# mantasu/face-crop-plus

Measured on AMD Instinct MI355X. Metric: faces/sec end-to-end (detect+align+crop), higher is better.
Workload: dtype f16x3; 1 GPU; RetinaFace detect + 5-pt align/crop, batch=32/GPU synthetic 1024x1024 RGB, strategy=largest, det_threshold=0.6, output 256x256, detector on 2 HIP streams x 16 images; global_batch=32, image_size=1024, parallelism=dp1

## Files before the change

### face-crop-plus_amd/csrc/fcp_bneck_chain.hip

```cpp
#include "fcp_conv_common.h"

#include <type_traits>

using namespace fcp_conv;

namespace {

typedef _Float16 f16x8 __attribute__((ext_vector_type(8)));

constexpr int FCP_CHAIN_STORE_AUX = 2;

struct ChainK {
  const float* t1;  unsigned t1_bytes;  int t1_ld;
  const float* w2;  unsigned w2_bytes;  const float* ws2;  const float* b2;
  const float* w3;  unsigned w3_bytes;  const float* ws3;  const float* b3;
  const float* res; int res_ld;
  float* out;       int out_ld;    unsigned out_bytes;
  const float* w1n; unsigned w1n_bytes; const float* ws1n; const float* b1n;
  float* t1n;       int t1n_ld;
  int n, h, w, M;
  int nt_store;
  int out_even;
  const float* t1b; unsigned t1b_bytes; int t1b_ld, hb, wb, sb;
};

constexpr int BMT = 128;
constexpr int C = 64;
constexpr int ROWB = 128;
constexpr int STAGE = (BMT + C) * ROWB;
constexpr int CT_OFF = 0;
constexpr int W1B_OFF = BMT * 128;
constexpr bool w1_double(int cn, bool has_c2) { return !has_c2 || W1B_OFF + 2 * cn * 128 + 2 * C * 128 <= 2 * STAGE; }
constexpr int w3b_off(int cn, bool has_c2) { return W1B_OFF + (w1_double(cn, has_c2) ? 2 : 1) * cn * 128; }
constexpr int r0_bytes(int cw, int cn, bool has_c2) { return has_c2 ? 2 * STAGE : w3b_off(cn, has_c2) + 2 * cw * 128; }
constexpr bool alias_t2(bool has_c2) { return !has_c2; }
constexpr int lds_bytes(int cw, int cn, bool has_c2, bool direct = false) {
  const int r0 = r0_bytes(cw, cn, has_c2), t2 = BMT * cw * 4;
  if (direct) return r0;
  return !alias_t2(has_c2) ? r0 + t2 : (r0 > W1B_OFF + t2 ? r0 : W1B_OFF + t2);
}
constexpr int wgs_per_cu(int cw, int cn, bool has_c2, bool direct = false) {
  if (direct) return cn == 0 && lds_bytes(cw, cn, has_c2, true) <= 80 * 1024 ? 2 : 1;
  return lds_bytes(cw, cn, has_c2) <= 80 * 1024 ? 2 : 1;
}

__device__ __forceinline__ int swz(int row) { return ((row >> 1) & 7) ^ ((row & 1) << 2); }

constexpr bool direct_form(int cn, int cw2) { return cw2 > 0 || cn == 0; }
template <int CN, int CW, int NOUT, bool HAS_C2, bool HAS_RES, int CW2 = 0>
__global__ void __launch_bounds__(2 * BMT, wgs_per_cu(CW, CN, HAS_C2, direct_form(CN, CW2))) bneck_chain_c64(const ChainK p) {
  constexpr bool DIRECT = direct_form(CN, CW2);
  static_assert(!DIRECT || (!HAS_C2 && CW2 % 32 == 0 && CW2 < CW), "direct forms are pair forms");
  constexpr bool HAS_P3 = CN > 0;
  static_assert(!HAS_C2 || CW == C, "phase 1 is written for 64-channel bottlenecks");
  constexpr bool PATCH = HAS_C2;
  constexpr int PH = BMT / 16;
  constexpr int NTHR = 2 * BMT;
  constexpr int NW = NTHR / 64;
  constexpr int LR = NTHR / 8;
  constexpr int TN3 = CN / 32;
  constexpr int TN3A = TN3 > 0 ? TN3 : 1;
  constexpr int CS = CW / 32;
  constexpr int NCH = NOUT / 32;
  constexpr int W3CH = CW * 128;
  constexpr bool ALIAS = alias_t2(HAS_C2) && !DIRECT;
  constexpr int T2_OFF = ALIAS ? W1B_OFF : r0_bytes(CW, CN, HAS_C2);
  constexpr int WGS = wgs_per_cu(CW, CN, HAS_C2, DIRECT);
  constexpr int WPS = WGS * NW / 4;
  static_assert(lds_bytes(CW, CN, HAS_C2, DIRECT) <= 160 * 1024, "LDS budget");
  constexpr bool W1DB = w1_double(CN, HAS_C2);
  constexpr bool SPREAD = W1DB && (HAS_C2 || WPS == 1);
  constexpr bool ROT = false;
  constexpr int PQ = ROT ? TN3 / CS : 0;
  static_assert(!ROT || (TN3 % CS == 0 && PQ >= 1), "rotated loop: TN3 must be a multiple of CS");
  constexpr bool W1PRE = !ROT && W1DB && !DIRECT && (HAS_C2 ? CN <= 64 || WPS == 1 : CN <= 128 && WPS == 1);
  constexpr int W3B_OFF = w3b_off(CN, HAS_C2);
  static_assert(!HAS_C2 || W3B_OFF + 2 * W3CH <= 2 * STAGE, "chunk buffers must fit the phase-1 stage region");
  constexpr int NRES = HAS_RES ? 4 : 0;
  extern __shared__ __attribute__((aligned(16))) float smem[];
  char* lds = reinterpret_cast<char*>(smem);

  const int nb = gridDim.x;
  const int bid = blockIdx.x;
  const int q8 = nb >> 3, r8 = nb & 7, xcd = bid & 7;
  const int tile_m = (xcd < r8 ? xcd * (q8 + 1) : r8 * (q8 + 1) + (xcd - r8) * q8) + (bid >> 3);

  const int tid = threadIdx.x;
  const int lane = tid & 63;
  const int wave = tid >> 6;
  const int wave_u = __builtin_amdgcn_readfirstlane(wave);
  const int lrow = tid >> 3;
  const int csrc = (tid & 7) ^ swz(lrow);
  const int l31 = lane & 31, half = lane >> 5;
  const int rsw = swz(l31);
  int offH[2], offL[2];
#pragma unroll
  for (int s = 0; s < 2; ++s) {
    offH[s] = ((2 * s + half) ^ rsw) << 4;
    offL[s] = ((4 + 2 * s + half) ^ rsw) << 4;
  }
// ... 33 lines not shown
      for (int e = 0; e < 8; ++e) {
        ws8[e] = p.ws2[ccol + e];
        b8[e] = p.b2[ccol + e];
      }
#pragma unroll
      for (int g = 0; g < 4; ++g) {
        const int row = (tid >> 3) + LR * g;
        const f32x4 a = *reinterpret_cast<const f32x4*>(Cs + row * C + ccol);
        const f32x4 b = *reinterpret_cast<const f32x4*>(Cs + row * C + ccol + 4);
        float v[8] = {a[0], a[1], a[2], a[3], b[0], b[1], b[2], b[3]};
#pragma unroll
        for (int e = 0; e < 8; ++e) v[e] = conv_value_relu(v[e], ws8[e], b8[e]);
        u32x4_t hi, lo;
        split8(f32x4{v[0], v[1], v[2], v[3]}, f32x4{v[4], v[5], v[6], v[7]}, hi, lo);
        const int q = (ccol & 31) >> 3, sw = swz(row);
        char* trow = lds + T2_OFF + (ccol >> 5) * (BMT * ROWB) + row * ROWB;
        *reinterpret_cast<u32x4_t*>(trow + ((q ^ sw) << 4)) = hi;
        *reinterpret_cast<u32x4_t*>(trow + (((4 + q) ^ sw) << 4)) = lo;
      }
    }
    __syncthreads();
  };

  if constexpr (HAS_C2) {
    constexpr int HALO = (PH + 2) * 18;
    constexpr int HROWS = (HALO + LR - 1) / LR * LR;
    constexpr int ASL = HROWS * ROWB;
    constexpr int TPB = 2, NSTEP = 18 / TPB;
    static_assert(18 % TPB == 0, "taps per barrier must divide the 18 K slices");
    constexpr int BST_OFF = 2 * ASL, BSL = C * ROWB, BSTG = TPB * BSL;
    static_assert(BST_OFF + 2 * BSTG <= T2_OFF + BMT * C * 4, "halo patch + filter stages must fit region 0 + T2");
    f32x16 acc1[2];
    const int wm = wave / 2, wn = wave % 2;
    __amdgpu_buffer_rsrc_t rs_in = __builtin_amdgcn_make_buffer_rsrc(const_cast<float*>(p.t1), 0, p.t1_bytes, 0x00020000);
    __amdgpu_buffer_rsrc_t rs_w = __builtin_amdgcn_make_buffer_rsrc(const_cast<float*>(p.w2), 0, p.w2_bytes, 0x00020000);
#pragma unroll
    for (int i = 0; i < HROWS / LR; ++i) {
      const int r = lrow + LR * i;
      const int hy = r / 18, hx = r - hy * 18;
      const int y = py0 - 1 + hy, x = px0 - 1 + hx;
      const bool ok = r < HALO && (unsigned)y < (unsigned)p.h && (unsigned)x < (unsigned)p.w;
      const unsigned src = ok ? ((unsigned)((pn * p.h + y) * p.w + x) * (unsigned)p.t1_ld + (unsigned)(csrc * 4)) * 4u : 0xFFFFFFFFu;
#pragma unroll
      for (int cs = 0; cs < 2; ++cs)
        __builtin_amdgcn_raw_ptr_buffer_load_lds(rs_in, (__attribute__((address_space(3))) void*)(lds + cs * ASL + (wave_u * 8 + LR * i) * ROWB), 16,
                                                 (int)(src == 0xFFFFFFFFu ? 0xFFFFFFFFu : src + (unsigned)(cs * 32 * 4)), 0, 0, 0);
    }
    constexpr int B_LD = C / LR;
    unsigned woff[B_LD];
#pragma unroll
    for (int i = 0; i < B_LD; ++i) woff[i] = (unsigned)(((lrow + LR * i) * (9 * C) + csrc * 4) * 4);
    auto dma_b = [&](int step, int stage) {
#pragma unroll
      for (int u = 0; u < TPB; ++u)
#pragma unroll
        for (int i = 0; i < B_LD; ++i)
          __builtin_amdgcn_raw_ptr_buffer_load_lds(rs_w, (__attribute__((address_space(3))) void*)(lds + BST_OFF + stage * BSTG + u * BSL + (wave_u * 8 + LR * i) * ROWB), 16,
                                                   (int)(woff[i] + (unsigned)((step * TPB + u) * BK * 4)), 0, 0, 0);
    };
    dma_b(0, 0);
#pragma unroll
    for (int i = 0; i < 2; ++i)
#pragma unroll
      for (int e = 0; e < 16; ++e) acc1[i][e] = 0.f;
    int hr0[2];
#pragma unroll
    for (int i = 0; i < 2; ++i) hr0[i] = (wm * 4 + i * 2 + (l31 >> 4)) * 18 + (l31 & 15);
    const char* Bw = lds + BST_OFF + (wn * 32 + l31) * ROWB;
    fcp_static_for<0, NSTEP>([&](auto gc) {
      constexpr int g = decltype(gc)::value;
// ... 21 lines not shown
          bl[sq] = *reinterpret_cast<const f16x8*>(Bb + offL[sq]);
        }
        if constexpr (decltype(uc)::value == TPB - 1) {
          asm volatile("s_waitcnt lgkmcnt(0)" ::: "memory");
          __builtin_amdgcn_sched_barrier(0);
          if constexpr (g + 1 < NSTEP) dma_b(g + 1, (g + 1) & 1);
          __builtin_amdgcn_sched_barrier(0);
        }
#pragma unroll
        for (int sq = 0; sq < 2; ++sq)
#pragma unroll
          for (int i = 0; i < 2; ++i) {
            acc1[i] = __builtin_amdgcn_mfma_f32_32x32x16_f16(al[sq][i], bh[sq], acc1[i], 0, 0, 0);
            acc1[i] = __builtin_amdgcn_mfma_f32_32x32x16_f16(ah[sq][i], bl[sq], acc1[i], 0, 0, 0);
            acc1[i] = __builtin_amdgcn_mfma_f32_32x32x16_f16(ah[sq][i], bh[sq], acc1[i], 0, 0, 0);
          }
        __builtin_amdgcn_sched_barrier(0);
      });
    });
    asm volatile("s_waitcnt vmcnt(0)" ::: "memory");
    __builtin_amdgcn_s_barrier();
    __builtin_amdgcn_sched_barrier(0);
    conv2_epilogue(acc1, wm, wn);
  } else if constexpr (!DIRECT) {
    __amdgpu_buffer_rsrc_t rs_in = __builtin_amdgcn_make_buffer_rsrc(const_cast<float*>(p.t1), 0, p.t1_bytes, 0x00020000);
#pragma unroll
    for (int i = 0; i < BMT / LR; ++i) {
      const int m = tile_m * BMT + lrow + LR * i;
      const unsigned ro = m < p.M ? ((unsigned)m * (unsigned)p.t1_ld + (unsigned)(csrc * 4)) * 4u : 0xFFFFFFFFu;
#pragma unroll
      for (int sl = 0; sl < CS; ++sl)
        __builtin_amdgcn_raw_ptr_buffer_load_lds(rs_in, (__attribute__((address_space(3))) void*)(lds + T2_OFF + sl * BMT * ROWB + wave_u * 8 * ROWB + LR * i * ROWB),
                                                 16, (int)(ro == 0xFFFFFFFFu ? 0xFFFFFFFFu : ro + (unsigned)(sl * 128)), 0, 0, 0);
    }
  }

  __amdgpu_buffer_rsrc_t rs_w3 = __builtin_amdgcn_make_buffer_rsrc(const_cast<float*>(p.w3), 0, p.w3_bytes, 0x00020000);
  __amdgpu_buffer_rsrc_t rs_w1 = __builtin_amdgcn_make_buffer_rsrc(const_cast<float*>(p.w1n), 0, p.w1n_bytes, 0x00020000);
  constexpr int PW3 = 4 * CS / NW;
  constexpr int PW1 = CN / (8 * NW);
  static_assert(PW3 >= 1 && (PW1 >= 1 || !HAS_P3), "filter pieces per wave");
  auto dma_w3 = [&](int j, int buf) {
#pragma unroll
    for (int i = 0; i < PW3; ++i) {
      const int g = wave_u * PW3 + i, sl = g >> 2, r = (g & 3) * 8 + (lane >> 3);
      char* dst = lds + W3B_OFF + buf * W3CH + sl * 4096 + (g & 3) * 8 * ROWB;
      const unsigned src = (unsigned)((j * 32 + r) * (CW * 4) + sl * 128 + (((lane & 7) ^ swz(r)) << 4));
      __builtin_amdgcn_raw_ptr_buffer_load_lds(rs_w3, (__attribute__((address_space(3))) void*)dst, 16, (int)src, 0, 0, 0);
    }
  };
  auto dma_w1 = [&](int j, int buf) {
    char* dst = lds + W1B_OFF + buf * (CN * ROWB) + wave_u * (CN / NW) * ROWB;
#pragma unroll
    for (int i = 0; i < PW1; ++i) {
      const int r = wave_u * (CN / NW) + 8 * i + (lane >> 3);
      const unsigned src = (unsigned)(r * (NOUT * 4) + j * 128 + (((lane & 7) ^ swz(r)) << 4));
      __builtin_amdgcn_raw_ptr_buffer_load_lds(rs_w1, (__attribute__((address_space(3))) void*)(dst + 8 * i * ROWB), 16, (int)src, 0, 0, 0);
    }
  };
  constexpr int NDMA = PW3 + PW1;
  auto dma_one = [&](auto kc, int j, int buf) {
    constexpr int k = decltype(kc)::value;
    if constexpr (k < PW3) {
      const int g = wave_u * PW3 + k, sl = g >> 2, r = (g & 3) * 8 + (lane >> 3);
      char* dst = lds + W3B_OFF + buf * W3CH + sl * 4096 + (g & 3) * 8 * ROWB;
      const unsigned src = (unsigned)((j * 32 + r) * (CW * 4) + sl * 128 + (((lane & 7) ^ swz(r)) << 4));
      __builtin_amdgcn_raw_ptr_buffer_load_lds(rs_w3, (__attribute__((address_space(3))) void*)dst, 16, (int)src, 0, 0, 0);
    } else {
      constexpr int i = k - PW3;
      const int j1 = ROT ? j - 1 : j, buf1 = ROT ? (j1 & 1) : buf;
      char* dst = lds + W1B_OFF + buf1 * (CN * ROWB) + wave_u * (CN / NW) * ROWB;
      const int r = wave_u * (CN / NW) + 8 * i + (lane >> 3);
      const unsigned src = (unsigned)(r * (NOUT * 4) + j1 * 128 + (((lane & 7) ^ swz(r)) << 4));
      __builtin_amdgcn_raw_ptr_buffer_load_lds(rs_w1, (__attribute__((address_space(3))) void*)(dst + 8 * i * ROWB), 16, (int)src, 0, 0, 0);
    }
  };

  f32x16 acc3[TN3A];
#pragma unroll
  for (int t = 0; t < TN3; ++t)
#pragma unroll
    for (int e = 0; e < 16; ++e) acc3[t][e] = 0.f;

  const char* a2base = lds + T2_OFF + (wave * 32 + l31) * ROWB;
  const char* a3base = lds + CT_OFF + (wave * 32 + l31) * ROWB;
  const int eq = lane & 3;
  const int erow0 = wave * 32 + (lane >> 2);
  long rm[2];
  unsigned so[2];
// ... 2 lines not shown
    const int prow = erow0 + 16 * it;
    const long m = pix(prow);
    rm[it] = m >= 0 ? m : (long)p.M - 1;
    const bool keep = !PATCH || !p.out_even || ((((prow >> 4) | prow) & 1) == 0);
    so[it] = (m >= 0 && keep) ? (unsigned)(m * p.out_ld * 4 + eq * 16) : 0xFFFFFFFFu;
  }
  __amdgpu_buffer_rsrc_t rs_out = __builtin_amdgcn_make_buffer_rsrc(p.out, 0, p.out_bytes, 0x00020000);

  u32x4_t rhi[2], rlo[2];
  auto load_res = [&](int j) {
    if constexpr (!HAS_RES) return;
#pragma unroll
    for (int it = 0; it < 2; ++it) {
      const char* pb = reinterpret_cast<const char*>(p.res) + rm[it] * p.res_ld * 4 + j * 128 + eq * 16;
      rhi[it] = *reinterpret_cast<const u32x4_t*>(pb);
      rlo[it] = *reinterpret_cast<const u32x4_t*>(pb + 64);
    }
  };
  const int nch = NCH;
  f16x8 pch[2], pcl[2];
  f16x8 wx[ROT ? TN3 : 1], wy[ROT ? TN3 : 1];
  float ws_l = p.ws3[l31], b_l = p.b3[l31];
  constexpr int NCONST = 2;
  f16x8 ah[CS][2], al[CS][2];
  auto read_a2 = [&]() {
#pragma unroll
    for (int sl = 0; sl < CS; ++sl)
#pragma unroll
      for (int s = 0; s < 2; ++s) {
        ah[sl][s] = *reinterpret_cast<const f16x8*>(a2base + sl * BMT * ROWB + offH[s]);
        al[sl][s] = *reinterpret_cast<const f16x8*>(a2base + sl * BMT * ROWB + offL[s]);
      }
  };
  if constexpr (DIRECT) {
    constexpr int CS1 = (CW - CW2) / 32;
    __amdgpu_buffer_rsrc_t rs_a = __builtin_amdgcn_make_buffer_rsrc(const_cast<float*>(p.t1), 0, p.t1_bytes, 0x00020000);
    __amdgpu_buffer_rsrc_t rs_b = __builtin_amdgcn_make_buffer_rsrc(const_cast<float*>(p.t1b), 0, p.t1b_bytes, 0x00020000);
    asm volatile("" ::: "memory");
    dma_w3(0, 0);
    if constexpr (W1DB && !ROT) dma_w1(0, 0);
    asm volatile("" ::: "memory");
    const long m = pix(wave * 32 + l31);
    unsigned oa = 0xFFFFFFFFu, ob = 0xFFFFFFFFu;
    if (m >= 0) {
      const int ni = (int)(m / hw);
      const int rem = (int)(m - (long)ni * hw);
      const int y = rem / p.w, x = rem - y * p.w;
      oa = (unsigned)m * (unsigned)p.t1_ld * 4u;
      ob = ((unsigned)(ni * p.hb + y * p.sb) * (unsigned)p.wb + (unsigned)(x * p.sb)) * (unsigned)p.t1b_ld * 4u;
    }
// ... 5 lines not shown
        const unsigned base = first ? oa : ob;
        const unsigned off = (unsigned)((first ? sl : sl - CS1) * 128);
        const unsigned vh = base == 0xFFFFFFFFu ? base : base + off + (unsigned)((2 * sk + half) << 4);
        const unsigned vl = base == 0xFFFFFFFFu ? base : base + off + (unsigned)((4 + 2 * sk + half) << 4);
        ah[sl][sk] = __builtin_bit_cast(f16x8, __builtin_amdgcn_raw_buffer_load_b128(first ? rs_a : rs_b, (int)vh, 0, 0));
        al[sl][sk] = __builtin_bit_cast(f16x8, __builtin_amdgcn_raw_buffer_load_b128(first ? rs_a : rs_b, (int)vl, 0, 0));
      }
    asm volatile("s_waitcnt vmcnt(0)" ::: "memory");
#pragma unroll
    for (int sl = 0; sl < CS; ++sl)
#pragma unroll
      for (int sk = 0; sk < 2; ++sk) asm volatile("" : "+v"(ah[sl][sk]), "+v"(al[sl][sk]));
    __builtin_amdgcn_sched_barrier(0);
  }
  if constexpr (ALIAS) {
    asm volatile("s_waitcnt vmcnt(0)" ::: "memory");
    __builtin_amdgcn_s_barrier();
    __builtin_amdgcn_sched_barrier(0);
    read_a2();
    asm volatile("s_waitcnt lgkmcnt(0)" ::: "memory");
    __builtin_amdgcn_s_barrier();
    __builtin_amdgcn_sched_barrier(0);
  }
  asm volatile("" ::: "memory");
  if constexpr (!DIRECT) {
    dma_w3(0, 0);
    if constexpr (W1DB && !ROT) dma_w1(0, 0);
  }
  asm volatile("" ::: "memory");
  if (nch > 0) load_res(0);
  __builtin_amdgcn_sched_barrier(0);

  for (int j = 0; j < nch; ++j) {
    const bool more = j + 1 < NCH;
    if (j == 0) asm volatile("s_waitcnt vmcnt(%0)" ::"n"(NRES) : "memory");
    else asm volatile("s_waitcnt vmcnt(%0)" ::"n"(4 + NCONST + NRES) : "memory");
    asm volatile("s_waitcnt lgkmcnt(0)" ::: "memory");
    __builtin_amdgcn_s_barrier();
    __builtin_amdgcn_sched_barrier(0);
    if constexpr (!SPREAD) {
      if (more) dma_w3(j + 1, (j + 1) & 1);
      if constexpr (W1DB) {
        if (more) dma_w1(j + 1, (j + 1) & 1);
      } else {
        dma_w1(j, 0);
      }
    }
    asm volatile("" ::: "memory");
    __builtin_amdgcn_sched_barrier(0);
    const char* b2base = lds + W3B_OFF + (j & 1) * W3CH + l31 * ROWB;
    if constexpr (!ALIAS && !DIRECT) {
      if (j == 0) read_a2();
    }
    constexpr int BG = (CS <= 4 && (HAS_C2 || WPS == 1)) ? CS : 2;
    f16x8 bh[2][BG][2], bl[2][BG][2];
    auto read_b2 = [&](int buf, int g) {
#pragma unroll
      for (int q = 0; q < BG; ++q)
#pragma unroll
        for (int s = 0; s < 2; ++s) {
          bh[buf][q][s] = *reinterpret_cast<const f16x8*>(b2base + (g * BG + q) * 4096 + offH[s]);
          bl[buf][q][s] = *reinterpret_cast<const f16x8*>(b2base + (g * BG + q) * 4096 + offL[s]);
        }
    };
    read_b2(0, 0);
    f16x8 dh[2][TN3A], dl[2][TN3A];
    if constexpr (W1PRE) {
      const char* w1b = lds + W1B_OFF + (j & 1) * (CN * ROWB);
#pragma unroll
      for (int s = 0; s < 2; ++s)
#pragma unroll
        for (int t = 0; t < TN3; ++t) {
          dh[s][t] = *reinterpret_cast<const f16x8*>(w1b + (t * 32 + l31) * ROWB + offH[s]);
          dl[s][t] = *reinterpret_cast<const f16x8*>(w1b + (t * 32 + l31) * ROWB + offL[s]);
// ... 210 lines not shown
      const f32x4 a = *reinterpret_cast<const f32x4*>(Cs + row * 64 + ccol);
      const f32x4 b = *reinterpret_cast<const f32x4*>(Cs + row * 64 + ccol + 4);
      float v[8] = {a[0], a[1], a[2], a[3], b[0], b[1], b[2], b[3]};
#pragma unroll
      for (int e = 0; e < 8; ++e) v[e] = conv_value_relu(v[e], ws8[e], b8[e]);
      if (m < 0) continue;
      u32x4_t hi, lo;
      split8(f32x4{v[0], v[1], v[2], v[3]}, f32x4{v[4], v[5], v[6], v[7]}, hi, lo);
      char* ob = reinterpret_cast<char*>(p.t1n) + m * p.t1n_ld * 4 + split_chan_off(co);
      if (p.nt_store) {
        __builtin_nontemporal_store(hi, reinterpret_cast<u32x4_t*>(ob));
        __builtin_nontemporal_store(lo, reinterpret_cast<u32x4_t*>(ob + 64));
      } else {
        *reinterpret_cast<u32x4_t*>(ob) = hi;
        *reinterpret_cast<u32x4_t*>(ob + 64) = lo;
      }
    }
    __syncthreads();
  }
}

template <int CN, int CW, int NOUT, bool HAS_C2, bool HAS_RES, int CW2 = 0>
int launch(const ChainK& k, hipStream_t s) {
  constexpr int LDS = lds_bytes(CW, CN, HAS_C2, direct_form(CN, CW2));
  FCP_LDS_OPT_IN((&bneck_chain_c64<CN, CW, NOUT, HAS_C2, HAS_RES, CW2>), LDS);
  const int tiles = HAS_C2 ? k.n * fcp_cdiv(k.h, BMT / 16) * ((k.w + 15) >> 4) : fcp_cdiv(k.M, BMT);
  hipLaunchKernelGGL((bneck_chain_c64<CN, CW, NOUT, HAS_C2, HAS_RES, CW2>), dim3(tiles), dim3(2 * BMT), LDS, s, k);
  FCP_LAUNCH_OK();
  return 0;
}

}

extern "C" int fcp_bottleneck_chain_f16x3(const fcp_chain_desc* d, fcp_stream_t stream) {
  FCP_REQUIRE(d != nullptr, "chain: null descriptor");
  const bool has_p3 = d->cn != 0 || d->w1n != nullptr;
  FCP_REQUIRE(d->t1 && d->w3 && d->ws3 && d->b3 && d->out && (!has_p3 || (d->w1n && d->ws1n && d->b1n && d->t1n)),
              "chain: null pointer (every convolution carries folded-BN bias and filter scales)");
  const bool has_c2 = d->w2 != nullptr;
  FCP_REQUIRE(!has_c2 || (d->ws2 && d->b2), "chain: conv2 needs its scales and bias");
  const int variant = (has_c2 && d->c == 64 && d->nout == 256 && d->res && (d->cn == 64 || d->cn == 128)) ? (d->cn == 64 ? 1 : 2)
                    : (!has_c2 && d->c == 128 && d->nout == 512 && d->res && d->cn == 128) ? 3
                    : (!has_c2 && d->c == 128 && d->nout == 256 && !d->res && d->cn == 64) ? 4
                    : (!has_c2 && d->c == 256 && d->nout == 1024 && d->res && d->cn == 256) ? 5
                    : (!has_c2 && d->c == 128 && d->nout == 512 && d->res && d->cn == 256) ? 6
                    : (!has_c2 && d->t1b && d->c == 384 && d->cb == 256 && d->nout == 512 && !d->res && d->cn == 128) ? 7
                    : (!has_c2 && !d->t1b && d->c == 256 && d->nout == 1024 && d->res && d->cn == 0 && !d->w1n) ? 8 : 0;
  FCP_REQUIRE(variant == 7 || !d->t1b, "chain: a second source (t1b) exists for the two-source pair form only (c 384 = 128 + 256, nout 512, cn 128)");
  FCP_REQUIRE(variant != 0, "chain: unsupported shape (c %d, conv2 %d, nout %d, residual %d, cn %d)", d->c, (int)has_c2, d->nout,
              d->res != nullptr, d->cn);
  FCP_REQUIRE(d->n > 0 && d->h > 0 && d->w > 0, "chain: bad sizes");
  const long M = (long)d->n * d->h * d->w;
  FCP_REQUIRE(M < (1L << 31), "chain: too many pixels");
  auto aligned = [](const void* p, int ld) { return ((uintptr_t)p & 127) == 0 && ld % 32 == 0; };
  FCP_REQUIRE(aligned(d->t1, d->t1_ld) && (!d->res || aligned(d->res, d->res_ld)) && aligned(d->out, d->out_ld) && (!has_p3 || aligned(d->t1n, d->t1n_ld)),
              "chain: tensors are split32 views: 128-byte aligned, channel stride a multiple of 32");
  FCP_REQUIRE(d->t1_ld >= d->c - (d->t1b ? d->cb : 0) && (!d->res || d->res_ld >= d->nout) && d->out_ld >= d->nout && (!has_p3 || d->t1n_ld >= d->cn), "chain: channel strides too small");
  const unsigned long t1_bytes = (unsigned long)M * d->t1_ld * 4ul;
  FCP_REQUIRE(t1_bytes < 0xFFFFFFF0ul, "chain: t1 must be below 4 GiB");
  ChainK k;
  k.t1 = d->t1; k.t1_bytes = (unsigned)t1_bytes; k.t1_ld = d->t1_ld;
  k.w2 = reinterpret_cast<const float*>(d->w2); k.w2_bytes = 128u * 9 * 64 * 4; k.ws2 = d->ws2; k.b2 = d->b2;
  k.w3 = reinterpret_cast<const float*>(d->w3); k.w3_bytes = (unsigned)(d->nout * d->c * 4); k.ws3 = d->ws3; k.b3 = d->b3;
  k.res = d->res; k.res_ld = d->res_ld; k.out = d->out; k.out_ld = d->out_ld;
  const unsigned long out_bytes = (unsigned long)M * d->out_ld * 4ul;
  FCP_REQUIRE(out_bytes < 0xFFFFFFF0ul, "chain: out must span less than 4 GiB");
  k.out_bytes = (unsigned)out_bytes;
  k.w1n = reinterpret_cast<const float*>(d->w1n); k.w1n_bytes = has_p3 ? (unsigned)(fcp_cdiv(d->cn, 128) * 128 * d->nout * 4) : 0u; k.ws1n = d->ws1n; k.b1n = d->b1n;
  k.t1n = d->t1n; k.t1n_ld = d->t1n_ld;
  k.n = d->n; k.h = d->h; k.w = d->w; k.M = (int)M;
  static const int nt_env = getenv("FCP_NT_STORE") ? atoi(getenv("FCP_NT_STORE")) : 1;
  k.nt_store = nt_env;
  k.t1b = nullptr; k.t1b_bytes = 0; k.t1b_ld = 0; k.hb = 0; k.wb = 0; k.sb = 1;
  if (d->t1b) {
    FCP_REQUIRE(aligned(d->t1b, d->t1b_ld) && d->t1b_ld >= d->cb && d->t1b_stride >= 1 && d->t1b_h > 0 && d->t1b_w > 0 &&
                (long)(d->h - 1) * d->t1b_stride < d->t1b_h && (long)(d->w - 1) * d->t1b_stride < d->t1b_w,
                "chain: t1b must be a split32 view whose (h, w) grid covers the output grid at t1b_stride");
    const unsigned long tb = (unsigned long)d->n * d->t1b_h * d->t1b_w * d->t1b_ld * 4ul;
    FCP_REQUIRE(tb < 0xFFFFFFF0ul, "chain: t1b must be below 4 GiB");
    k.t1b = d->t1b; k.t1b_bytes = (unsigned)tb; k.t1b_ld = d->t1b_ld; k.hb = d->t1b_h; k.wb = d->t1b_w; k.sb = d->t1b_stride;
  }
  k.out_even = (d->flags & FCP_CHAIN_OUT_EVEN_ONLY) ? 1 : 0;
  FCP_REQUIRE(!k.out_even || has_c2, "chain: FCP_CHAIN_OUT_EVEN_ONLY needs a conv2 form");
  hipStream_t s = (hipStream_t)stream;
  switch (variant) {
    case 1: return launch<64, 64, 256, true, true>(k, s);
    case 2: return launch<128, 64, 256, true, true>(k, s);
    case 3: return launch<128, 128, 512, false, true>(k, s);
    case 5: return launch<256, 256, 1024, false, true>(k, s);
    case 6: return launch<256, 128, 512, false, true>(k, s);
    case 7: return launch<128, 384, 512, false, false, 256>(k, s);
    case 8: return launch<0, 256, 1024, false, true>(k, s);
    default: return launch<64, 128, 256, false, false>(k, s);
  }
}
```

### face-crop-plus_amd/engine.py

```python
from __future__ import annotations

import contextlib
import ctypes as C
import os
import threading
from dataclasses import dataclass

import numpy as np
import torch

from . import _native as N
from . import torch_ops as T

BN_EPS = 1e-5
COUT_PAD = 128


class Act:
    __slots__ = ("buf", "c0", "c", "fmt")

    def __init__(self, buf: torch.Tensor, c0: int = 0, c: int | None = None, fmt: int = 0):
        assert buf.dim() == 4 and buf.dtype == torch.float32 and buf.is_contiguous()
        self.buf, self.c0, self.fmt = buf, c0, fmt
        self.c = buf.shape[3] - c0 if c is None else c
# ... 630 lines not shown
        head = f"conv {pc.kh}x{pc.kw} s{pc.stride} {pc.cin}->{pc.cout} @{oh}x{ow}"
        return (f"{head} tile {tm}x{tn}{' bal' if flags & N.CONV_BALANCE_TAIL else ''}{' +res' if res1 is not None else ''}",
                head, pc.flops_per_pixel * m, byts)

    def relaunch(o):
        o = _alias_safe_out(o, x, x2, res1, res2)
        return "fcp_conv2d_nhwc_f32", (C.byref(desc(o)),), (pc, x, x2, res1, res2, o)
    return _accounted(go, describe, relaunch)[0]


def tile_candidates(cout: int, halo_ok: bool, wide_ok: bool, big_ok: bool):
    cands = [(128, 128), (128, 64)]
    if halo_ok:
        cands = ([(128, 32)] if cout <= 32 else []) + [(128, 64), (1, 32)]
    if wide_ok:
        cands = cands + [(1, 128)]
    if big_ok:
        big = [(256, 128)] + ([(256, 256)] if cout >= 256 else []) + ([(256, 192)] if 128 < cout <= 192 else [])
        cands += big
        cands += [(tm, tn, N.CONV_BALANCE_TAIL) for tm, tn in big]
    return cands


def chain_supported(pc2: PackedConv | None, pc3: PackedConv, pc1n: PackedConv | None, residual: bool = True, cb: int = 0) -> bool:
    convs = [pc for pc in (pc2, pc3, pc1n) if pc is not None]
    if not all(pc.precision == 1 and pc.bias is not None and not pc.cin4 for pc in convs):
        return False
    one = lambda pc, cin, cout: (pc.cin, pc.cout, pc.kh, pc.kw, pc.stride, pc.pad) == (cin, cout, 1, 1, 1, 0)
    if pc1n is None:
        return pc2 is None and residual and not cb and one(pc3, 256, 1024)
    if cb:
        return pc2 is None and not residual and cb == 256 and one(pc3, 384, 512) and one(pc1n, 512, 128)
    if pc2 is not None:
        return ((pc2.cin, pc2.cout, pc2.kh, pc2.kw, pc2.stride, pc2.pad) == (64, 64, 3, 3, 1, 1) and residual
                and one(pc3, 64, 256) and (one(pc1n, 256, 64) or one(pc1n, 256, 128)))
    if residual:
        return ((one(pc3, 128, 512) and (one(pc1n, 512, 128) or one(pc1n, 512, 256)))
                or (one(pc3, 256, 1024) and one(pc1n, 1024, 256)))
    return one(pc3, 128, 256) and one(pc1n, 256, 64)



def _chain_desc(pc2, pc3, pc1n, t1, res, out, t1n, tile_m, flags, t1b, t1b_stride) -> N.ChainDesc:
    d = N.ChainDesc()
    d.t1, d.res, d.out = t1.ptr(), (res.ptr() if res is not None else None), out.ptr()
    d.t1n = t1n.ptr() if t1n is not None else None
    d.w2, d.ws2, d.b2 = map(N.ptr, _filter(pc2))
    d.w3, d.ws3, d.b3 = map(N.ptr, _filter(pc3))
    d.w1n, d.ws1n, d.b1n = map(N.ptr, _filter(pc1n))
    d.n, d.h, d.w, d.c, d.nout = t1.n, t1.h, t1.w, pc3.cin, pc3.cout
    d.cn = pc1n.cout if pc1n is not None else 0
    d.t1_ld, d.res_ld, d.out_ld = t1.ld, (res.ld if res is not None else 0), out.ld
    d.t1n_ld = t1n.ld if t1n is not None else 0
    d.tile_m, d.flags = tile_m, flags
    if t1b is not None:
        d.t1b, d.cb, d.t1b_ld, d.t1b_h, d.t1b_w, d.t1b_stride = t1b.ptr(), t1b.c, t1b.ld, t1b.h, t1b.w, t1b_stride
    return d


def bottleneck_chain(pc2: PackedConv | None, pc3: PackedConv, pc1n: PackedConv, t1: Act, res: Act | None,
                     out: Act | None = None, t1n: Act | None = None, tile_m: int = 0, out_even_only: bool = False,
                     t1b: Act | None = None, t1b_stride: int = 1):
    cb = t1b.c if t1b is not None else 0
    assert chain_supported(pc2, pc3, pc1n, res is not None, cb), "bottleneck_chain: unsupported shapes"
    assert t1.fmt == 1 and t1.c + cb == pc3.cin and (res is None or (res.fmt == 1 and res.c == pc3.cout))
    assert t1b is None or (t1b.fmt == 1 and t1b.n == t1.n and (t1.h - 1) * t1b_stride < t1b.h and (t1.w - 1) * t1b_stride < t1b.w)
    assert res is None or (t1.n, t1.h, t1.w) == (res.n, res.h, res.w)
    c, nout, cn = pc3.cin, pc3.cout, (pc1n.cout if pc1n is not None else 0)
    flags = N.CHAIN_OUT_EVEN_ONLY if (out_even_only and pc2 is not None and RangeMonitor.active is None) else 0
    via_op = T.ENABLED and out is None and t1n is None
    if not via_op:
        if out is None:
            out = Act.empty(t1.n, t1.h, t1.w, nout, t1.buf.device, 1)
        if t1n is None and pc1n is not None:
            t1n = Act.empty(t1.n, t1.h, t1.w, cn, t1.buf.device, 1)
        assert out.fmt == 1 and (out.n, out.h, out.w, out.c) == (t1.n, t1.h, t1.w, nout)
        assert pc1n is None or (t1n.fmt == 1 and (t1n.n, t1n.h, t1n.w, t1n.c) == (t1.n, t1.h, t1.w, cn))
    desc = lambda o, o1n: _chain_desc(pc2, pc3, pc1n, t1, res, o, o1n, tile_m, flags, t1b, t1b_stride)

    def go():
        if not via_op:
            _c_launch("fcp_bottleneck_chain_f16x3", C.byref(desc(out, t1n)))
            return out, t1n
        o, t = T.load().bottleneck_chain(t1.buf, t1.c0, None if res is None else res.buf, 0 if res is None else res.c0,
                                         *_filter(pc2), *_filter(pc3), *_filter(pc1n), c, nout, cn, tile_m, flags,
                                         None if t1b is None else t1b.buf, 0 if t1b is None else t1b.c0, cb, int(t1b_stride))
        return Act(o, fmt=1), (Act(t, fmt=1) if pc1n is not None else None)

    def describe():
        m = t1.n * t1.h * t1.w
        flops = ((pc2.flops_per_pixel if pc2 is not None else 0) + pc3.flops_per_pixel
                 + (pc1n.flops_per_pixel if pc1n is not None else 0)) * m
        byts = 4 * (m * (c + (nout if not flags else nout // 4) + (nout if res is not None else 0) + cn) + (0 if pc2 is None else 9 * c * c)
                    + c * nout + nout * cn)
        if pc1n is None:
            head = f"expand {c}->{nout} @{t1.h}x{t1.w}"
            return f"{head} +res", head, flops, byts
        head = f"chain {'3x3 ' if pc2 is not None else ''}{c}->{nout}->{cn} @{t1.h}x{t1.w}"
        return (f"{head}{' +res' if res is not None else ''}{' out@even' if flags else ''}{' two-source' if t1b is not None else ''}",
                head, flops, byts)

    def relaunch(o, o1n):
        o = _alias_safe_out(o, t1, res, t1b)
        o1n = o1n if o1n is None else _alias_safe_out(o1n, t1, res, t1b)
        return "fcp_bottleneck_chain_f16x3", (C.byref(desc(o, o1n)),), (pc2, pc3, pc1n, t1, res, o, o1n, t1b)
    return _accounted(go, describe, relaunch)


def u8_to_nhwc4(images_u8: torch.Tensor, sub=(0.0, 0.0, 0.0), div: float = 1.0) -> Act:
    assert images_u8.dtype == torch.uint8 and images_u8.dim() == 4 and images_u8.shape[3] == 3
    assert images_u8.is_contiguous()
    n, h, w, _ = images_u8.shape
    out = Act.empty(n, h, w, 4, images_u8.device)
    sub_arr = (C.c_float * 3)(*[float(s) for s in sub])
    N.check(N.lib().fcp_u8_to_nhwc4_f32(N.ptr(images_u8), out.ptr(), n * h * w, sub_arr, float(div),
                                        N.stream_ptr()), "fcp_u8_to_nhwc4_f32")
    return out


@dataclass
class PackedStem:
    wfrag: torch.Tensor
    bias: torch.Tensor
    wscale: torch.Tensor
    flops_per_pixel: int


def pack_stem_fused(weight, bn, device, cin_perm=None) -> PackedStem:
    if isinstance(weight, torch.Tensor):
# ... 131 lines not shown
```

### face-crop-plus_amd/retinaface.py

```python
from __future__ import annotations


import os
import threading

import numpy as np
import torch

from . import _native as N
from . import engine as E
from . import torch_ops as T
from .weights import load_state_dict

STRATEGIES = {"all": 0, "best": 1, "largest": 2}


class RetinaFace:
    WEIGHTS_FILENAME = "retinaface_detector.pth"

    def __init__(self, strategy: str = "all", vis: float = 0.6):
        self.strategy = strategy
        self.vis_threshold = vis
        self.nms_threshold = 0.4
        self.variance = [0.1, 0.2]
        self.device = None
        self._p = None
        self.precision = 0
        self.fused_chain = True
        self.streams = int(os.environ.get("FCP_DET_STREAMS", "2"))
        self.min_images_per_stream = 6
        self._tls = threading.local()

    def load(self, device: str | torch.device = "cuda:0", weights=None, precision=None):
        device = torch.device(device)
        if device.type != "cuda":
            raise RuntimeError("face_crop_plus_amd runs on an AMD GPU only (device must be cuda:N / hip); "
                               "there is no CPU fallback")
        N.lib()
        self.device = device
        sd = load_state_dict("retinaface", weights, device=device)
        self._repack(sd, precision)
        E.device_props(device)
        E.selfcheck_at_load(self, sd, weights, precision, lambda: self._repack(sd, "f32"))
        return self

    def _repack(self, sd, precision):
        with torch.cuda.device(self.device), E.default_precision(precision):
            self._p = self._pack(sd, self.device)
        self.precision = E.resolve_precision(precision)

    @torch.no_grad()
# ... 65 lines not shown
            p[f"fpn.merge{i}"] = pc(sd[f"fpn.merge{i}.0.weight"], None, bn(sd, f"fpn.merge{i}.1"), 1, 1, dev)
        head_perm = list(range(0, 128)) + list(range(192, 256)) + list(range(128, 192))
        for k in (1, 2, 3):
            def folded(nm):
                return E.fold_bn(sd[f"ssh{k}.{nm}.0.weight"].numpy(), {q: v.numpy() for q, v in bn(sd, f"ssh{k}.{nm}.1").items()}, None)
            w_b, b_b = folded("conv5X5_1")
            w_a, b_a = folded("conv3X3")
            p[f"ssh{k}.ab"] = pc(np.concatenate([w_b, w_a]), np.concatenate([b_b, b_a]), None, 1, 1, dev)
            w_c, b_c = folded("conv5X5_2")
            w_d, b_d = folded("conv7X7_2")
            p[f"ssh{k}.cd"] = pc(np.concatenate([w_c, w_d]), np.concatenate([b_c, b_d]), None, 1, 1, dev)
            w_e, b_e = folded("conv7x7_3")
            p[f"ssh{k}.e"] = pc(w_e, b_e, None, 1, 1, dev)
            i = k - 1
            hw = np.concatenate([sd[f"{h}.{i}.conv1x1.weight"].numpy() for h in ("ClassHead", "BboxHead", "LandmarkHead")])
            hb = np.concatenate([sd[f"{h}.{i}.conv1x1.bias"].numpy() for h in ("ClassHead", "BboxHead", "LandmarkHead")])
            p[f"head{k}"] = pc(hw, hb, None, 1, 0, dev, cin_perm=head_perm)
        return p

    def forward_heads(self, x4: E.Act | None, images_u8: torch.Tensor | None = None, heads_out=None):
        p = self._p
        f = 1 if self.precision == 1 else 0
        stem_t1 = None
        if images_u8 is not None and "stem_fused" in p:
            n, h, w, _ = images_u8.shape
            hp, wp = ((h - 1) // 2) // 2 + 1, ((w - 1) // 2) // 2 + 1
            cat = E.Act.empty(n, hp, wp, 128, images_u8.device, f)
            c1 = p["blocks"][0]["c1"]
            if f == 1 and E.stem_conv1_supported(c1):
                x, stem_t1 = E.stem_relu_pool_u8(p["stem_fused"], images_u8, cat.slice(64, 64), conv1=c1)
            else:
                x = E.stem_relu_pool_u8(p["stem_fused"], images_u8, cat.slice(64, 64))
        else:
            x = E.conv(p["stem"], x4, act_slope=0.0, out_fmt=f)
            cat = E.Act.empty(x.n, (x.h + 1) // 2, (x.w + 1) // 2, 2 * x.c, x.buf.device, f)
            x = E.maxpool3x3s2(x, cat.slice(x.c, x.c))
        feats = []
        blocks, pre = p["blocks"], stem_t1
        chain = bool(f) and self.fused_chain
        for bi, blk in enumerate(blocks):
            o = pre if pre is not None else E.conv(blk["c1"], x, act_slope=0.0, out_fmt=f)
            pre = None
            nxt = blocks[bi + 1] if bi + 1 < len(blocks) else None
            if (chain and blk["ds"] is None and not blk["feat"] and nxt is not None
                    and E.chain_supported(blk["c2"], blk["c3"], nxt["c1"])):
                sparse = "c3ds" in nxt and nxt["c2"].stride == 2 and not blk["feat"]
                x, pre = E.bottleneck_chain(blk["c2"], blk["c3"], nxt["c1"], o, x, out_even_only=sparse)
                continue
            if "c3ds" in blk and blk["c2"].stride == 1:
                E.conv(blk["c2"], o, cat.slice(0, o.c), act_slope=0.0)
                if chain and nxt is not None and E.chain_supported(None, blk["c3ds"], nxt["c1"], residual=False):
                    x, pre = E.bottleneck_chain(None, blk["c3ds"], nxt["c1"], cat, None)
                else:
                    x = E.conv(blk["c3ds"], cat, act_slope=0.0, out_fmt=f)
                del cat
                continue
            if "c3ds" in blk:
                o = E.conv(blk["c2"], o, act_slope=0.0, out_fmt=f)
                if (chain and not blk["feat"] and nxt is not None
                        and E.chain_supported(None, blk["c3ds"], nxt["c1"], residual=False, cb=x.c)):
                    x, pre = E.bottleneck_chain(None, blk["c3ds"], nxt["c1"], o, None, t1b=x, t1b_stride=blk["c2"].stride)
                    continue
                x = E.conv(blk["c3ds"], o, act_slope=0.0, out_fmt=f, x2=x, x2_stride=blk["c2"].stride)
                if blk["feat"]:
                    feats.append(x)
                continue
            o = E.conv(blk["c2"], o, act_slope=0.0, out_fmt=f)
            if (chain and blk["ds"] is None and nxt is not None and E.chain_supported(None, blk["c3"], nxt["c1"])):
                x, pre = E.bottleneck_chain(None, blk["c3"], nxt["c1"], o, x)
                if blk["feat"]:
# ... 207 lines not shown
```

Before: 1435 faces/s.

## Fuse first bottleneck's conv2 and concat-downsample into a two-source entry chain kernel

Adds an entry form of the bottleneck chain kernel that runs the 3x3 conv2, then the 1x1 c3ds over the concatenation of the conv2 output and the pooled stem output (read directly from global as a second source), then the next block's conv1. This drops the separate conv2 launch, the write and re-read of the 128-channel concat buffer, and the standalone c3ds. In exchange it adds register pressure from holding the second-source fragments across phase 1, and it places the second W3 filter buffer in the head of the T2 region. The path is on by default and can be disabled with an environment flag.

After: 1443 faces/s (median of 6 runs). No clear change (+0.6%).

```diff
diff --git a/face-crop-plus_amd/csrc/fcp_bneck_chain.hip b/face-crop-plus_amd/csrc/fcp_bneck_chain.hip
--- a/face-crop-plus_amd/csrc/fcp_bneck_chain.hip
+++ b/face-crop-plus_amd/csrc/fcp_bneck_chain.hip
@@ -46,11 +46,14 @@
 
 __device__ __forceinline__ int swz(int row) { return ((row >> 1) & 7) ^ ((row & 1) << 2); }
 
-constexpr bool direct_form(int cn, int cw2) { return cw2 > 0 || cn == 0; }
+constexpr bool direct_form(int cn, int cw2, bool has_c2) { return !has_c2 && (cw2 > 0 || cn == 0); }
 template <int CN, int CW, int NOUT, bool HAS_C2, bool HAS_RES, int CW2 = 0>
-__global__ void __launch_bounds__(2 * BMT, wgs_per_cu(CW, CN, HAS_C2, direct_form(CN, CW2))) bneck_chain_c64(const ChainK p) {
-  constexpr bool DIRECT = direct_form(CN, CW2);
-  static_assert(!DIRECT || (!HAS_C2 && CW2 % 32 == 0 && CW2 < CW), "direct forms are pair forms");
+__global__ void __launch_bounds__(2 * BMT, wgs_per_cu(CW, CN, HAS_C2, direct_form(CN, CW2, HAS_C2))) bneck_chain_c64(const ChainK p) {
+  constexpr bool DIRECT = direct_form(CN, CW2, HAS_C2);
+  static_assert(!DIRECT || (CW2 % 32 == 0 && CW2 < CW), "direct pair forms: CW counts both sources");
+  constexpr bool ENTRY = HAS_C2 && CW2 > 0;
+  static_assert(!ENTRY || (CW2 % 32 == 0 && !HAS_RES && CN == 64), "entry form: 64 + CW2 -> NOUT -> 64, no residual");
+  constexpr int KT = ENTRY ? CW + CW2 : CW;
   constexpr bool HAS_P3 = CN > 0;
   static_assert(!HAS_C2 || CW == C, "phase 1 is written for 64-channel bottlenecks");
   constexpr bool PATCH = HAS_C2;
@@ -60,22 +63,25 @@
   constexpr int LR = NTHR / 8;
   constexpr int TN3 = CN / 32;
   constexpr int TN3A = TN3 > 0 ? TN3 : 1;
-  constexpr int CS = CW / 32;
+  constexpr int CS = KT / 32;
+  constexpr int CSL = ENTRY ? CW / 32 : CS;
   constexpr int NCH = NOUT / 32;
-  constexpr int W3CH = CW * 128;
+  constexpr int W3CH = KT * 128;
+  constexpr bool W3_IN_T2 = ENTRY;
   constexpr bool ALIAS = alias_t2(HAS_C2) && !DIRECT;
   constexpr int T2_OFF = ALIAS ? W1B_OFF : r0_bytes(CW, CN, HAS_C2);
   constexpr int WGS = wgs_per_cu(CW, CN, HAS_C2, DIRECT);
   constexpr int WPS = WGS * NW / 4;
   static_assert(lds_bytes(CW, CN, HAS_C2, DIRECT) <= 160 * 1024, "LDS budget");
   constexpr bool W1DB = w1_double(CN, HAS_C2);
-  constexpr bool SPREAD = W1DB && (HAS_C2 || WPS == 1);
+  constexpr bool SPREAD = W1DB && ((HAS_C2 && !ENTRY) || WPS == 1);
   constexpr bool ROT = false;
   constexpr int PQ = ROT ? TN3 / CS : 0;
   static_assert(!ROT || (TN3 % CS == 0 && PQ >= 1), "rotated loop: TN3 must be a multiple of CS");
-  constexpr bool W1PRE = !ROT && W1DB && !DIRECT && (HAS_C2 ? CN <= 64 || WPS == 1 : CN <= 128 && WPS == 1);
+  constexpr bool W1PRE = !ROT && W1DB && !DIRECT && !ENTRY && (HAS_C2 ? CN <= 64 || WPS == 1 : CN <= 128 && WPS == 1);
   constexpr int W3B_OFF = w3b_off(CN, HAS_C2);
-  static_assert(!HAS_C2 || W3B_OFF + 2 * W3CH <= 2 * STAGE, "chunk buffers must fit the phase-1 stage region");
+  static_assert(!HAS_C2 || W3B_OFF + 2 * W3CH <= 2 * STAGE + (W3_IN_T2 ? BMT * CW * 4 : 0), "chunk buffers must fit the phase-1 stage region");
+  static_assert(!W3_IN_T2 || (W1DB && W3B_OFF + W3CH == T2_OFF), "entry form: the second filter buffer is the head of T2");
   constexpr int NRES = HAS_RES ? 4 : 0;
   extern __shared__ __attribute__((aligned(16))) float smem[];
   char* lds = reinterpret_cast<char*>(smem);
@@ -155,6 +161,7 @@
     __syncthreads();
   };
 
+  f16x8 ah[CS][2], al[CS][2];
   if constexpr (HAS_C2) {
     constexpr int HALO = (PH + 2) * 18;
     constexpr int HROWS = (HALO + LR - 1) / LR * LR;
@@ -179,6 +186,23 @@
         __builtin_amdgcn_raw_ptr_buffer_load_lds(rs_in, (__attribute__((address_space(3))) void*)(lds + cs * ASL + (wave_u * 8 + LR * i) * ROWB), 16,
                                                  (int)(src == 0xFFFFFFFFu ? 0xFFFFFFFFu : src + (unsigned)(cs * 32 * 4)), 0, 0, 0);
     }
+    if constexpr (ENTRY) {
+      __amdgpu_buffer_rsrc_t rs_b = __builtin_amdgcn_make_buffer_rsrc(const_cast<float*>(p.t1b), 0, p.t1b_bytes, 0x00020000);
+      const int prow = wave * 32 + l31;
+      const int y = py0 + (prow >> 4), x = px0 + (prow & 15);
+      const unsigned ob = (y < p.h && x < p.w)
+                              ? ((unsigned)((pn * p.hb + y * p.sb) * p.wb + x * p.sb) * (unsigned)p.t1b_ld) * 4u : 0xFFFFFFFFu;
+#pragma unroll
+      for (int sl = CSL; sl < CS; ++sl)
+#pragma unroll
+        for (int sk = 0; sk < 2; ++sk) {
+          const unsigned off = (unsigned)((sl - CSL) * 128);
+          const unsigned vh = ob == 0xFFFFFFFFu ? ob : ob + off + (unsigned)((2 * sk + half) << 4);
+          const unsigned vl = ob == 0xFFFFFFFFu ? ob : ob + off + (unsigned)((4 + 2 * sk + half) << 4);
+          ah[sl][sk] = __builtin_bit_cast(f16x8, __builtin_amdgcn_raw_buffer_load_b128(rs_b, (int)vh, 0, 0));
+          al[sl][sk] = __builtin_bit_cast(f16x8, __builtin_amdgcn_raw_buffer_load_b128(rs_b, (int)vl, 0, 0));
+        }
+    }
     constexpr int B_LD = C / LR;
     unsigned woff[B_LD];
 #pragma unroll
@@ -246,6 +270,13 @@
     __builtin_amdgcn_s_barrier();
     __builtin_amdgcn_sched_barrier(0);
     conv2_epilogue(acc1, wm, wn);
+    if constexpr (ENTRY) {
+#pragma unroll
+      for (int sl = CSL; sl < CS; ++sl)
+#pragma unroll
+        for (int sk = 0; sk < 2; ++sk) asm volatile("" : "+v"(ah[sl][sk]), "+v"(al[sl][sk]));
+      __builtin_amdgcn_sched_barrier(0);
+    }
   } else if constexpr (!DIRECT) {
     __amdgpu_buffer_rsrc_t rs_in = __builtin_amdgcn_make_buffer_rsrc(const_cast<float*>(p.t1), 0, p.t1_bytes, 0x00020000);
 #pragma unroll
@@ -269,7 +300,7 @@
     for (int i = 0; i < PW3; ++i) {
       const int g = wave_u * PW3 + i, sl = g >> 2, r = (g & 3) * 8 + (lane >> 3);
       char* dst = lds + W3B_OFF + buf * W3CH + sl * 4096 + (g & 3) * 8 * ROWB;
-      const unsigned src = (unsigned)((j * 32 + r) * (CW * 4) + sl * 128 + (((lane & 7) ^ swz(r)) << 4));
+      const unsigned src = (unsigned)((j * 32 + r) * (KT * 4) + sl * 128 + (((lane & 7) ^ swz(r)) << 4));
       __builtin_amdgcn_raw_ptr_buffer_load_lds(rs_w3, (__attribute__((address_space(3))) void*)dst, 16, (int)src, 0, 0, 0);
     }
   };
@@ -288,7 +319,7 @@
     if constexpr (k < PW3) {
       const int g = wave_u * PW3 + k, sl = g >> 2, r = (g & 3) * 8 + (lane >> 3);
       char* dst = lds + W3B_OFF + buf * W3CH + sl * 4096 + (g & 3) * 8 * ROWB;
-      const unsigned src = (unsigned)((j * 32 + r) * (CW * 4) + sl * 128 + (((lane & 7) ^ swz(r)) << 4));
+      const unsigned src = (unsigned)((j * 32 + r) * (KT * 4) + sl * 128 + (((lane & 7) ^ swz(r)) << 4));
       __builtin_amdgcn_raw_ptr_buffer_load_lds(rs_w3, (__attribute__((address_space(3))) void*)dst, 16, (int)src, 0, 0, 0);
     } else {
       constexpr int i = k - PW3;
@@ -337,10 +368,9 @@
   f16x8 wx[ROT ? TN3 : 1], wy[ROT ? TN3 : 1];
   float ws_l = p.ws3[l31], b_l = p.b3[l31];
   constexpr int NCONST = 2;
-  f16x8 ah[CS][2], al[CS][2];
   auto read_a2 = [&]() {
 #pragma unroll
-    for (int sl = 0; sl < CS; ++sl)
+    for (int sl = 0; sl < CSL; ++sl)
 #pragma unroll
       for (int s = 0; s < 2; ++s) {
         ah[sl][s] = *reinterpret_cast<const f16x8*>(a2base + sl * BMT * ROWB + offH[s]);
@@ -392,6 +422,12 @@
     __builtin_amdgcn_s_barrier();
     __builtin_amdgcn_sched_barrier(0);
   }
+  if constexpr (W3_IN_T2) {
+    read_a2();
+    asm volatile("s_waitcnt lgkmcnt(0)" ::: "memory");
+    __builtin_amdgcn_s_barrier();
+    __builtin_amdgcn_sched_barrier(0);
+  }
   asm volatile("" ::: "memory");
   if constexpr (!DIRECT) {
     dma_w3(0, 0);
@@ -419,7 +455,7 @@
     asm volatile("" ::: "memory");
     __builtin_amdgcn_sched_barrier(0);
     const char* b2base = lds + W3B_OFF + (j & 1) * W3CH + l31 * ROWB;
-    if constexpr (!ALIAS && !DIRECT) {
+    if constexpr (!ALIAS && !DIRECT && !W3_IN_T2) {
       if (j == 0) read_a2();
     }
     constexpr int BG = (CS <= 4 && (HAS_C2 || WPS == 1)) ? CS : 2;
@@ -676,7 +712,7 @@
 
 template <int CN, int CW, int NOUT, bool HAS_C2, bool HAS_RES, int CW2 = 0>
 int launch(const ChainK& k, hipStream_t s) {
-  constexpr int LDS = lds_bytes(CW, CN, HAS_C2, direct_form(CN, CW2));
+  constexpr int LDS = lds_bytes(CW, CN, HAS_C2, direct_form(CN, CW2, HAS_C2));
   FCP_LDS_OPT_IN((&bneck_chain_c64<CN, CW, NOUT, HAS_C2, HAS_RES, CW2>), LDS);
   const int tiles = HAS_C2 ? k.n * fcp_cdiv(k.h, BMT / 16) * ((k.w + 15) >> 4) : fcp_cdiv(k.M, BMT);
   hipLaunchKernelGGL((bneck_chain_c64<CN, CW, NOUT, HAS_C2, HAS_RES, CW2>), dim3(tiles), dim3(2 * BMT), LDS, s, k);
@@ -699,8 +735,11 @@
                     : (!has_c2 && d->c == 256 && d->nout == 1024 && d->res && d->cn == 256) ? 5
                     : (!has_c2 && d->c == 128 && d->nout == 512 && d->res && d->cn == 256) ? 6
                     : (!has_c2 && d->t1b && d->c == 384 && d->cb == 256 && d->nout == 512 && !d->res && d->cn == 128) ? 7
-                    : (!has_c2 && !d->t1b && d->c == 256 && d->nout == 1024 && d->res && d->cn == 0 && !d->w1n) ? 8 : 0;
-  FCP_REQUIRE(variant == 7 || !d->t1b, "chain: a second source (t1b) exists for the two-source pair form only (c 384 = 128 + 256, nout 512, cn 128)");
+                    : (!has_c2 && !d->t1b && d->c == 256 && d->nout == 1024 && d->res && d->cn == 0 && !d->w1n) ? 8
+                    : (has_c2 && d->t1b && d->c == 128 && d->cb == 64 && d->nout == 256 && !d->res && d->cn == 64 && d->t1b_stride == 1) ? 9 : 0;
+  FCP_REQUIRE(variant == 7 || variant == 9 || !d->t1b,
+              "chain: a second source (t1b) exists for the two-source pair form (c 384 = 128 + 256, nout 512, cn 128) and the entry form "
+              "(conv2, c 128 = 64 + 64, nout 256, no residual, cn 64, t1b_stride 1) only");
   FCP_REQUIRE(variant != 0, "chain: unsupported shape (c %d, conv2 %d, nout %d, residual %d, cn %d)", d->c, (int)has_c2, d->nout,
               d->res != nullptr, d->cn);
   FCP_REQUIRE(d->n > 0 && d->h > 0 && d->w > 0, "chain: bad sizes");
@@ -735,7 +774,7 @@
     k.t1b = d->t1b; k.t1b_bytes = (unsigned)tb; k.t1b_ld = d->t1b_ld; k.hb = d->t1b_h; k.wb = d->t1b_w; k.sb = d->t1b_stride;
   }
   k.out_even = (d->flags & FCP_CHAIN_OUT_EVEN_ONLY) ? 1 : 0;
-  FCP_REQUIRE(!k.out_even || has_c2, "chain: FCP_CHAIN_OUT_EVEN_ONLY needs a conv2 form");
+  FCP_REQUIRE(!k.out_even || (has_c2 && variant != 9), "chain: FCP_CHAIN_OUT_EVEN_ONLY needs a conv2 form with a residual (not the entry form)");
   hipStream_t s = (hipStream_t)stream;
   switch (variant) {
     case 1: return launch<64, 64, 256, true, true>(k, s);
@@ -745,6 +784,7 @@
     case 6: return launch<256, 128, 512, false, true>(k, s);
     case 7: return launch<128, 384, 512, false, false, 256>(k, s);
     case 8: return launch<0, 256, 1024, false, true>(k, s);
+    case 9: return launch<64, 64, 256, true, false, 64>(k, s);
     default: return launch<64, 128, 256, false, false>(k, s);
   }
 }
diff --git a/face-crop-plus_amd/engine.py b/face-crop-plus_amd/engine.py
--- a/face-crop-plus_amd/engine.py
+++ b/face-crop-plus_amd/engine.py
@@ -676,13 +676,17 @@
     return cands
 
 
-def chain_supported(pc2: PackedConv | None, pc3: PackedConv, pc1n: PackedConv | None, residual: bool = True, cb: int = 0) -> bool:
+def chain_supported(pc2: PackedConv | None, pc3: PackedConv, pc1n: PackedConv | None, residual: bool = True, cb: int = 0,
+                    t1b_stride: int = 1, out_even_only: bool = False) -> bool:
     convs = [pc for pc in (pc2, pc3, pc1n) if pc is not None]
     if not all(pc.precision == 1 and pc.bias is not None and not pc.cin4 for pc in convs):
         return False
     one = lambda pc, cin, cout: (pc.cin, pc.cout, pc.kh, pc.kw, pc.stride, pc.pad) == (cin, cout, 1, 1, 1, 0)
     if pc1n is None:
         return pc2 is None and residual and not cb and one(pc3, 256, 1024)
+    if cb and pc2 is not None:
+        return ((pc2.cin, pc2.cout, pc2.kh, pc2.kw, pc2.stride, pc2.pad) == (64, 64, 3, 3, 1, 1) and not residual
+                and cb == 64 and t1b_stride == 1 and not out_even_only and one(pc3, 128, 256) and one(pc1n, 256, 64))
     if cb:
         return pc2 is None and not residual and cb == 256 and one(pc3, 384, 512) and one(pc1n, 512, 128)
     if pc2 is not None:
@@ -715,8 +719,12 @@
 def bottleneck_chain(pc2: PackedConv | None, pc3: PackedConv, pc1n: PackedConv, t1: Act, res: Act | None,
                      out: Act | None = None, t1n: Act | None = None, tile_m: int = 0, out_even_only: bool = False,
                      t1b: Act | None = None, t1b_stride: int = 1):
+    return _bottleneck_chain(pc2, pc3, pc1n, t1, res, out, t1n, tile_m, out_even_only, t1b, t1b_stride)
+
+
+def _bottleneck_chain(pc2, pc3, pc1n, t1, res, out, t1n, tile_m, out_even_only, t1b, t1b_stride):
     cb = t1b.c if t1b is not None else 0
-    assert chain_supported(pc2, pc3, pc1n, res is not None, cb), "bottleneck_chain: unsupported shapes"
+    assert chain_supported(pc2, pc3, pc1n, res is not None, cb, t1b_stride, out_even_only), "bottleneck_chain: unsupported shapes"
     assert t1.fmt == 1 and t1.c + cb == pc3.cin and (res is None or (res.fmt == 1 and res.c == pc3.cout))
     assert t1b is None or (t1b.fmt == 1 and t1b.n == t1.n and (t1.h - 1) * t1b_stride < t1b.h and (t1.w - 1) * t1b_stride < t1b.w)
     assert res is None or (t1.n, t1.h, t1.w) == (res.n, res.h, res.w)
@@ -745,7 +753,8 @@
         m = t1.n * t1.h * t1.w
         flops = ((pc2.flops_per_pixel if pc2 is not None else 0) + pc3.flops_per_pixel
                  + (pc1n.flops_per_pixel if pc1n is not None else 0)) * m
-        byts = 4 * (m * (c + (nout if not flags else nout // 4) + (nout if res is not None else 0) + cn) + (0 if pc2 is None else 9 * c * c)
+        byts = 4 * (m * (c + (nout if not flags else nout // 4) + (nout if res is not None else 0) + cn)
+                    + (0 if pc2 is None else 9 * pc2.cin * pc2.cout)
                     + c * nout + nout * cn)
         if pc1n is None:
             head = f"expand {c}->{nout} @{t1.h}x{t1.w}"
@@ -759,6 +768,11 @@
         o1n = o1n if o1n is None else _alias_safe_out(o1n, t1, res, t1b)
         return "fcp_bottleneck_chain_f16x3", (C.byref(desc(o, o1n)),), (pc2, pc3, pc1n, t1, res, o, o1n, t1b)
     return _accounted(go, describe, relaunch)
+
+
+def bottleneck_chain_entry(pc2: PackedConv, pc3: PackedConv, pc1n: PackedConv, t1: Act, t1b: Act,
+                           out: Act | None = None, t1n: Act | None = None):
+    return _bottleneck_chain(pc2, pc3, pc1n, t1, None, out, t1n, 0, False, t1b, 1)
 
 
 def u8_to_nhwc4(images_u8: torch.Tensor, sub=(0.0, 0.0, 0.0), div: float = 1.0) -> Act:
diff --git a/face-crop-plus_amd/retinaface.py b/face-crop-plus_amd/retinaface.py
--- a/face-crop-plus_amd/retinaface.py
+++ b/face-crop-plus_amd/retinaface.py
@@ -27,6 +27,7 @@
         self._p = None
         self.precision = 0
         self.fused_chain = True
+        self.fused_entry = os.environ.get("FCP_DET_ENTRY", "1") != "0"
         self.streams = int(os.environ.get("FCP_DET_STREAMS", "2"))
         self.min_images_per_stream = 6
         self._tls = threading.local()
@@ -138,22 +139,26 @@
         p = self._p
         f = 1 if self.precision == 1 else 0
         stem_t1 = None
+        blocks = p["blocks"]
+        chain = bool(f) and self.fused_chain
+        entry = (chain and self.fused_entry and "c3ds" in blocks[0]
+                 and E.chain_supported(blocks[0]["c2"], blocks[0]["c3ds"], blocks[1]["c1"], residual=False, cb=64))
         if images_u8 is not None and "stem_fused" in p:
             n, h, w, _ = images_u8.shape
             hp, wp = ((h - 1) // 2) // 2 + 1, ((w - 1) // 2) // 2 + 1
-            cat = E.Act.empty(n, hp, wp, 128, images_u8.device, f)
-            c1 = p["blocks"][0]["c1"]
+            cat = E.Act.empty(n, hp, wp, 64 if entry else 128, images_u8.device, f)
+            pooled = cat if entry else cat.slice(64, 64)
+            c1 = blocks[0]["c1"]
             if f == 1 and E.stem_conv1_supported(c1):
-                x, stem_t1 = E.stem_relu_pool_u8(p["stem_fused"], images_u8, cat.slice(64, 64), conv1=c1)
+                x, stem_t1 = E.stem_relu_pool_u8(p["stem_fused"], images_u8, pooled, conv1=c1)
             else:
-                x = E.stem_relu_pool_u8(p["stem_fused"], images_u8, cat.slice(64, 64))
+                x = E.stem_relu_pool_u8(p["stem_fused"], images_u8, pooled)
         else:
             x = E.conv(p["stem"], x4, act_slope=0.0, out_fmt=f)
-            cat = E.Act.empty(x.n, (x.h + 1) // 2, (x.w + 1) // 2, 2 * x.c, x.buf.device, f)
-            x = E.maxpool3x3s2(x, cat.slice(x.c, x.c))
+            cat = E.Act.empty(x.n, (x.h + 1) // 2, (x.w + 1) // 2, x.c if entry else 2 * x.c, x.buf.device, f)
+            x = E.maxpool3x3s2(x, cat if entry else cat.slice(x.c, x.c))
         feats = []
-        blocks, pre = p["blocks"], stem_t1
-        chain = bool(f) and self.fused_chain
+        pre = stem_t1
         for bi, blk in enumerate(blocks):
             o = pre if pre is not None else E.conv(blk["c1"], x, act_slope=0.0, out_fmt=f)
             pre = None
@@ -162,6 +167,10 @@
                     and E.chain_supported(blk["c2"], blk["c3"], nxt["c1"])):
                 sparse = "c3ds" in nxt and nxt["c2"].stride == 2 and not blk["feat"]
                 x, pre = E.bottleneck_chain(blk["c2"], blk["c3"], nxt["c1"], o, x, out_even_only=sparse)
+                continue
+            if "c3ds" in blk and blk["c2"].stride == 1 and entry:
+                x, pre = E.bottleneck_chain_entry(blk["c2"], blk["c3ds"], nxt["c1"], o, x)
+                del cat
                 continue
             if "c3ds" in blk and blk["c2"].stride == 1:
                 E.conv(blk["c2"], o, cat.slice(0, o.c), act_slope=0.0)
```
